# lucidrains/progen

Measured on NVIDIA H100. Metric: tokens_per_sec, higher is better.
Workload: dtype bf16

## Files before the change

### include/progen_b200.h

```cpp
#ifndef PROGEN_B200_H
#define PROGEN_B200_H
#include <stdint.h>

#ifdef __cplusplus
extern "C" {
#endif

#define PROGEN_F32 0
#define PROGEN_BF16 1

#define PROGEN_BACKEND_SIMT 0
#define PROGEN_BACKEND_TC 1

#define PROGEN_EPI_STORE 0
#define PROGEN_EPI_ROTARY 1
#define PROGEN_EPI_RESIDUAL 2
#define PROGEN_EPI_GLU 3
#define PROGEN_EPI_GELU 4
#define PROGEN_EPI_GLU_BWD 5
#define PROGEN_EPI_GELU_BWD 6
#define PROGEN_EPI_ACCUM 7

const char* progen_version(void);
const char* progen_last_error(void);
int progen_device_check(void);
long long progen_launch_count(void);

typedef struct progen_gemm_t {
  int32_t M, N, K;
  int32_t a_mn_major, b_mn_major;
  int32_t batch;
  int32_t batch_reduce;
  int32_t causal;
  int32_t split_k;
  int32_t in_dtype, out_dtype, epi_kind, backend;
  int32_t seq_len, dim_head;
  int32_t atomic, tril, tril_rows;
  int64_t lda, ldb;
  int64_t a_batch_rows, b_batch_rows, d_batch_rows;
  int64_t ldo, ldo2, ldaux;
  const void* A;
  const void* B;
  void* out;
  void* out2;
  const float* bias;
  const void* aux;
  const float* rot_sin;
  const float* rot_cos;
  float* colsum;
  int64_t lda2, ldb2;
  const void* A2;
  const void* B2;
  int32_t K2, a2_mn_major, b2_mn_major, _pad_tail;
} progen_gemm_t;

int progen_gemm(const progen_gemm_t* desc, void* stream);

int progen_embed_fwd(const int* tokens, const float* table, float* x, long long T, int d, int V, void* stream);
int progen_embed_bwd(const int* tokens, const float* dx, float* dtable, long long T, int d, int V, void* stream);

int progen_ln_shift_fwd(const void* x, long long ldx, int x_dtype, const float* scale, void* y, long long ldy, int y_dtype,
                        float* mean, float* rstd, long long T, int d, int seq_len, int shift, void* stream);
int progen_ln_shift_bwd(const void* dy, long long lddy, int act_dtype, const void* x, long long ldx, int x_dtype,
                        const float* scale, const float* mean, const float* rstd, float* dres, void* dout, long long ldo,
                        float* dscale, float* dres_colsum, long long T, int d, int seq_len, int shift, int residual,
                        void* stream);

int progen_colsum(const void* in, long long ld, int dtype, float* out, long long T, int N, void* stream);

int progen_ce_fwd_bwd(const void* logits, int dtype, const int* labels, float* weights, float* loss, void* dlogits,
                      int dlogits_dtype, int B, int n, int V, float inv_batch, void* stream);

int progen_token_logprob(const void* logits, int dtype, const int* labels, float* logp, float* seq_ll, float* seq_count,
                         int B, int n, int V, void* stream);
int progen_preference_head(const void* logits, int dtype, const int* labels, const float* ref_ll, float* logp, float* seq_ll,
                           float* seq_count, float* weights, float* stats, float* loss, float* ce_scratch, void* dlogits,
                           int dlogits_dtype, int pairs, int n, int V, float beta, float inv_pairs, void* stream);
int progen_masked_mean_pool(const void* x, long long ldx, int dtype, const int* labels, float* out, int B, int n, int d,
                            void* stream);
int progen_masked_mean_pool_bwd(const float* demb, const int* labels, void* dy, long long ldy, int dtype, int B, int n, int d,
                                void* stream);

#define PROGEN_PROPERTY_MAX_OUTPUTS 64
#define PROGEN_TASK_REGRESSION 0
#define PROGEN_TASK_CLASSIFICATION 1
int progen_property_head(const float* emb, const float* w, const float* bias, int B, int d, int C, int task, const float* y,
                         const int* cls, float inv_batch, float* pred, float* row_loss, float* loss, float* dpred, float* dw,
                         float* db, float* demb, void* stream);

// ... 121 lines not shown
```

### progen_b200/csrc/api.cu

```cuda
#include <stdarg.h>
#include "gemm.h"
#include "../../include/progen_b200.h"

static thread_local char g_err[1024] = "";
unsigned long long g_progen_launches = 0;

void progen_set_error(const char* fmt, ...) {
  va_list ap;
  va_start(ap, fmt);
  vsnprintf(g_err, sizeof(g_err), fmt, ap);
  va_end(ap);
}

extern "C" {

const char* progen_version(void) { return "progen_b200 0.1.0 (sm_90a; wgmma/TMA GEMM, CUDA " CUDA_VERSION_STR ")"; }

const char* progen_last_error(void) { return g_err; }

long long progen_launch_count(void) { return (long long)__atomic_load_n(&g_progen_launches, __ATOMIC_RELAXED); }

int progen_device_check(void) {
  int dev = 0;
  PG_CUDA(cudaGetDevice(&dev));
  cudaDeviceProp prop;
  PG_CUDA(cudaGetDeviceProperties(&prop, dev));
  if (prop.major != 9) {
    progen_set_error("device %d (%s) is sm_%d%d; libprogen_b200 is built for sm_90a only", dev, prop.name, prop.major,
                     prop.minor);
    return PROGEN_ERR_DEVICE;
  }
  return PROGEN_OK;
}

int progen_gemm(const progen_gemm_t* d, void* stream) {
  PG_CHECK_ARG(d != nullptr);
  GemmArgs g;
  g.M = d->M; g.N = d->N; g.K = d->K;
  g.A = d->A; g.lda = d->lda; g.a_mn_major = d->a_mn_major;
  g.B = d->B; g.ldb = d->ldb; g.b_mn_major = d->b_mn_major;
  g.batch = d->batch < 1 ? 1 : d->batch;
  g.a_batch_rows = d->a_batch_rows; g.b_batch_rows = d->b_batch_rows; g.d_batch_rows = d->d_batch_rows;
  g.batch_reduce = d->batch_reduce; g.causal = d->causal; g.split_k = d->split_k < 1 ? 1 : d->split_k;
  g.in_dtype = d->in_dtype; g.out_dtype = d->out_dtype; g.epi_kind = d->epi_kind;
  g.epi.out = d->out; g.epi.ldo = d->ldo; g.epi.out2 = d->out2; g.epi.ldo2 = d->ldo2;
  g.epi.bias = d->bias; g.epi.aux = d->aux; g.epi.ldaux = d->ldaux;
  g.epi.rot_sin = d->rot_sin; g.epi.rot_cos = d->rot_cos;
  g.epi.seq_len = d->seq_len > 0 ? d->seq_len : 1; g.epi.dim_head = d->dim_head > 0 ? d->dim_head : 2;
  g.epi.atomic = d->atomic; g.epi.tril = d->tril; g.epi.tril_rows = d->tril_rows > 0 ? d->tril_rows : 1;
  g.epi.colsum = d->colsum;
  g.K2 = d->K2;
  g.A2 = d->A2; g.lda2 = d->lda2; g.a2_mn_major = d->a2_mn_major;
  g.B2 = d->B2; g.ldb2 = d->ldb2; g.b2_mn_major = d->b2_mn_major;
  PG_CHECK_ARG(g.epi_kind >= 0 && g.epi_kind < EPI_NUM_KINDS);
  PG_CHECK_ARG(g.epi.out != nullptr);
  PG_CHECK_ARG(!g.epi.colsum || g.epi_kind == EPI_GLU_BWD || g.epi_kind == EPI_GELU_BWD);
  if (g.epi_kind == EPI_GLU || g.epi_kind == EPI_GELU) PG_CHECK_ARG(g.epi.bias != nullptr);
  if (g.epi_kind == EPI_GLU_BWD || g.epi_kind == EPI_GELU_BWD) PG_CHECK_ARG(g.epi.aux != nullptr);
  if (g.epi_kind == EPI_ROTARY) PG_CHECK_ARG(g.epi.rot_sin && g.epi.rot_cos && d->seq_len > 0 && d->dim_head > 0 && d->dim_head % 2 == 0);
  if (d->backend == PROGEN_BACKEND_TC) return gemm_tc_launch(g, (cudaStream_t)stream);
  if (d->backend == PROGEN_BACKEND_SIMT) return gemm_simt_launch(g, (cudaStream_t)stream);
  progen_set_error("progen_gemm: unknown backend %d", d->backend);
  return PROGEN_ERR_ARG;
}

}
```

### progen_b200/csrc/gemm.h

```cpp
#pragma once
#include "epilogues.cuh"

struct GemmArgs {
  int M, N, K;
  const void* A; long long lda; int a_mn_major;
  const void* B; long long ldb; int b_mn_major;
  int batch; long long a_batch_rows; long long b_batch_rows; long long d_batch_rows;
  int batch_reduce;
  int causal;
  int split_k;
  int in_dtype;
  int out_dtype;
  int epi_kind;
  EpiArgs epi;
  const void* A2; long long lda2; int a2_mn_major;
  const void* B2; long long ldb2; int b2_mn_major;
  int K2;
};

#define PG_CHECK_TAIL(a)                                                                                               \
  do {                                                                                                                 \
    PG_CHECK_ARG((a).K2 >= 0);                                                                                         \
    if ((a).K2 > 0) {                                                                                                  \
      PG_CHECK_ARG((a).A2 != nullptr && (a).B2 != nullptr);                                                            \
      PG_CHECK_ARG((a).split_k == 1 && !(a).causal && (a).batch == 1 && !(a).batch_reduce && (a).epi_kind != EPI_ACCUM); \
    }                                                                                                                  \
  } while (0)

int gemm_tc_launch(const GemmArgs& g, cudaStream_t stream);
int gemm_simt_launch(const GemmArgs& g, cudaStream_t stream);
```

### progen_b200/csrc/gemm_tc.cu

```cuda
#include <cuda.h>
#include <algorithm>
#include <mutex>
#include <unordered_map>
#include "gemm.h"
#include "tc_ptx.cuh"

namespace {

using namespace tc;

constexpr int BM = 128;
constexpr int BN = 128;
constexpr int BK = 64;
constexpr int WG_K = 16;
constexpr int THREADS = 384;
constexpr int A_BYTES = BM * BK * 2;
constexpr int B_BYTES = BN * BK * 2;
constexpr int STAGE_BYTES = A_BYTES + B_BYTES;
constexpr int STAGES = 4;
constexpr int EPI_ROWS = 64;
constexpr int EPI_ITEMS = EPI_ROWS * (BN / 8) / 128;
constexpr int CS_LD = BN + 4;
constexpr int CS_BYTES = EPI_ROWS * CS_LD * 4;
constexpr int SMEM_TOTAL = 1024  + STAGES * STAGE_BYTES + 2 * CS_BYTES + 2 * STAGES * 8;
static_assert(SMEM_TOTAL <= 227 * 1024, "H100: 227 KiB of shared memory per block");
constexpr int BAR_TURN = 1, BAR_EPI = 3;
constexpr int PRODUCER_REGS = 40, CONSUMER_REGS = 232;
static_assert(128 * PRODUCER_REGS + 256 * CONSUMER_REGS <= 65536, "register file");

__device__ __forceinline__ void named_bar_sync(int id, int n) { asm volatile("bar.sync %0, %1;" ::"r"(id), "r"(n) : "memory"); }
__device__ __forceinline__ void named_bar_arrive(int id, int n) { asm volatile("bar.arrive %0, %1;" ::"r"(id), "r"(n) : "memory"); }
template <int R> __device__ __forceinline__ void setmaxnreg_dec() { asm volatile("setmaxnreg.dec.sync.aligned.u32 %0;" ::"n"(R)); }
template <int R> __device__ __forceinline__ void setmaxnreg_inc() { asm volatile("setmaxnreg.inc.sync.aligned.u32 %0;" ::"n"(R)); }

struct GemmDev {
  int M, N, K;
  int batch, batch_reduce;
  int a_batch_rows, b_batch_rows;
  long long d_batch_rows;
  int causal, split_k;
  EpiArgs epi;
  int K2;
};

struct TileInfo {
  int z, m0, n0, kb_begin, kb_end;
  int kb_main;
};

template <bool TAIL>
__device__ __forceinline__ void decode_tile(const GemmDev& g, int t, TileInfo& ti) {
  const int m_tiles = (g.M + BM - 1) / BM;
  const int n_tiles = (g.N + BN - 1) / BN;
  const int per_z = g.split_k * m_tiles * n_tiles;
  ti.z = t / per_z;
  int r = t - ti.z * per_z;
  const int ks = r / (m_tiles * n_tiles);
  r -= ks * (m_tiles * n_tiles);
  ti.m0 = (r / n_tiles) * BM;
  ti.n0 = (r % n_tiles) * BN;
  const int kb_total = (g.K + BK - 1) / BK;
  int b = 0, e = kb_total;
  if (g.causal == 1) e = min(kb_total, (ti.m0 + BM + BK - 1) / BK);
  if (g.causal == 2) b = min(kb_total, ti.m0 / BK);
  if (g.split_k > 1) {
    const int per = (kb_total + g.split_k - 1) / g.split_k;
    b = min(kb_total, ks * per);
    e = min(kb_total, b + per);
  }
  ti.kb_begin = b;
  ti.kb_end = e;
  if constexpr (TAIL) {
    ti.kb_main = e;
    ti.kb_end = e + (g.K2 + BK - 1) / BK;
  }
}

template <bool A_MN, bool B_MN, int KIND, typename TO, bool TAIL>
__global__ void __launch_bounds__(THREADS, 1)
gemm_tc_kernel(const __grid_constant__ CUtensorMap tma_a, const __grid_constant__ CUtensorMap tma_b,
               const __grid_constant__ CUtensorMap tma_a2, const __grid_constant__ CUtensorMap tma_b2, const GemmDev g,
               const int tiles) {
  extern __shared__ uint8_t smem_raw[];
  const uint32_t raw_u32 = smem_u32(smem_raw);
  const uint32_t smem_base = (raw_u32 + 1023u) & ~1023u;
  const uint32_t cs_base = smem_base + STAGES * STAGE_BYTES;
  const uint32_t bar_base = cs_base + 2 * CS_BYTES;
  auto full_bar = [&](int s) { return bar_base + 8u * s; };
  auto empty_bar = [&](int s) { return bar_base + 8u * (STAGES + s); };

  const int wg = threadIdx.x >> 7;
  if (threadIdx.x == 0) {
    prefetch_tensormap(&tma_a);
    prefetch_tensormap(&tma_b);
    if constexpr (TAIL) {
      prefetch_tensormap(&tma_a2);
// ... 152 lines not shown
        const float4 x0 = *reinterpret_cast<const float4*>(cs + r * CS_LD + cc);
        const float4 x1 = *reinterpret_cast<const float4*>(cs + r * CS_LD + cc + 4);
        v[0] = x0.x; v[1] = x0.y; v[2] = x0.z; v[3] = x0.w; v[4] = x1.x; v[5] = x1.y; v[6] = x1.z; v[7] = x1.w;
        epi_finish<KIND, TO, 8>(g.epi, row_first + EPI_ROWS * h + 8 * i, col, v, cb, pre[i], col_ok && m < g.M, csum);
        if (h == 0)
          epi_load<KIND, TO, 8>(g.epi, row_first + EPI_ROWS + 8 * i, col, col_ok && m + EPI_ROWS < g.M, pre[i]);
      }
    }
    if constexpr (CS::W > 0) {
      if (g.epi.colsum) {
        constexpr int TW = 16 * CS::W;
#pragma unroll
        for (int k = 0; k < CS::W; ++k) csum[k] += __shfl_xor_sync(0xffffffffu, csum[k], 16);
        named_bar_sync(BAR_EPI + c, 128);
        if (lane < 16) {
#pragma unroll
          for (int k = 0; k < CS::W; k += 4)
            *reinterpret_cast<float4*>(cs + w * TW + lane * CS::W + k) = make_float4(csum[k], csum[k + 1], csum[k + 2], csum[k + 3]);
        }
        named_bar_sync(BAR_EPI + c, 128);
        const int out0 = CS::OUT_SCALE * ti.n0, out_cols = CS::OUT_SCALE * g.N;
#pragma unroll
        for (int q = tid; q < TW / 4; q += 128) {
          float4 s = *reinterpret_cast<const float4*>(cs + 4 * q);
#pragma unroll
          for (int ww = 1; ww < 4; ++ww) {
            const float4 x = *reinterpret_cast<const float4*>(cs + ww * TW + 4 * q);
            s.x += x.x; s.y += x.y; s.z += x.z; s.w += x.w;
          }
          if (out0 + 4 * q < out_cols)
            asm volatile("red.global.add.v4.f32 [%0], {%1, %2, %3, %4};" ::"l"(g.epi.colsum + out0 + 4 * q), "f"(s.x),
                         "f"(s.y), "f"(s.z), "f"(s.w) : "memory");
        }
      }
    }
  }
}

typedef CUresult (*EncodeTiledFn)(CUtensorMap*, CUtensorMapDataType, cuuint32_t, void*, const cuuint64_t*,
                                  const cuuint64_t*, const cuuint32_t*, const cuuint32_t*, CUtensorMapInterleave,
                                  CUtensorMapSwizzle, CUtensorMapL2promotion, CUtensorMapFloatOOBfill);

EncodeTiledFn get_encode_fn() {
  static EncodeTiledFn fn = nullptr;
  static std::once_flag once;
  std::call_once(once, [] {
    void* p = nullptr;
    cudaDriverEntryPointQueryResult q;
    if (cudaGetDriverEntryPoint("cuTensorMapEncodeTiled", &p, cudaEnableDefault, &q) == cudaSuccess &&
        q == cudaDriverEntryPointSuccess)
      fn = reinterpret_cast<EncodeTiledFn>(p);
  });
  return fn;
}

struct MapKey {
  const void* ptr; uint64_t inner, outer, stride; uint32_t box_inner, box_outer, elem_bytes, swizzle;
  bool operator==(const MapKey& o) const {
    return ptr == o.ptr && inner == o.inner && outer == o.outer && stride == o.stride && box_inner == o.box_inner &&
           box_outer == o.box_outer && elem_bytes == o.elem_bytes && swizzle == o.swizzle;
  }
};
struct MapKeyHash {
  size_t operator()(const MapKey& k) const {
    size_t h = std::hash<const void*>()(k.ptr);
    auto mix = [&](uint64_t v) { h ^= std::hash<uint64_t>()(v) + 0x9e3779b97f4a7c15ULL + (h << 6) + (h >> 2); };
// ... 19 lines not shown
  cuuint32_t box[2] = {box_inner, box_outer};
  cuuint32_t estr[2] = {1, 1};
  CUtensorMap m;
  CUresult r = fn(&m, elem_bytes == 4 ? CU_TENSOR_MAP_DATA_TYPE_FLOAT32 : CU_TENSOR_MAP_DATA_TYPE_BFLOAT16, 2,
                  const_cast<void*>(ptr), dims, strides, box, estr, CU_TENSOR_MAP_INTERLEAVE_NONE, sw, CU_TENSOR_MAP_L2_PROMOTION_L2_256B,
                  CU_TENSOR_MAP_FLOAT_OOB_FILL_NONE);
  if (r != CUDA_SUCCESS) {
    progen_set_error("cuTensorMapEncodeTiled failed (CUresult %d) ptr=%p inner=%llu outer=%llu stride=%llu box=%ux%u", (int)r,
                     ptr, (unsigned long long)inner, (unsigned long long)outer, (unsigned long long)row_stride_elems,
                     box_inner, box_outer);
    return PROGEN_ERR_CUDA;
  }
  if (cache.size() > 4096) cache.clear();
  cache.emplace(key, m);
  *out = m;
  return PROGEN_OK;
}


template <bool A_MN, bool B_MN, int KIND, typename TO, bool TAIL>
int launch_inst(const CUtensorMap& ta, const CUtensorMap& tb, const CUtensorMap& ta2, const CUtensorMap& tb2,
                const GemmDev& gd, int tiles, cudaStream_t stream) {
  auto kern = gemm_tc_kernel<A_MN, B_MN, KIND, TO, TAIL>;
  static bool attr_set = false;
  if (!attr_set) {
    PG_CUDA(cudaFuncSetAttribute(kern, cudaFuncAttributeMaxDynamicSharedMemorySize, SMEM_TOTAL));
    attr_set = true;
  }
  kern<<<std::min(tiles, pg_num_sms()), THREADS, SMEM_TOTAL, stream>>>(ta, tb, ta2, tb2, gd, tiles);
  PG_LAUNCH_CHECK();
  return PROGEN_OK;
}

}

int pg_tensor_map_2d_bf16(const void* ptr, uint64_t inner, uint64_t outer, uint64_t row_stride_elems, uint32_t box_inner,
                          uint32_t box_outer, CUtensorMap* out) {
  return get_tensor_map(ptr, inner, outer, row_stride_elems, box_inner, box_outer, out);
}

int gemm_tc_launch(const GemmArgs& a, cudaStream_t stream) {
  PG_CHECK_ARG(a.in_dtype == PG_BF16);
  PG_CHECK_ARG(a.M > 0 && a.N > 0 && a.K > 0 && a.batch >= 1 && a.split_k >= 1);
  PG_CHECK_ARG(a.N % 8 == 0);
  PG_CHECK_ARG(a.K % BK == 0);
  PG_CHECK_ARG(a.lda % 8 == 0 && a.ldb % 8 == 0);
  PG_CHECK_ARG((reinterpret_cast<uintptr_t>(a.A) & 15) == 0 && (reinterpret_cast<uintptr_t>(a.B) & 15) == 0);
  PG_CHECK_ARG(!(a.split_k > 1 && a.causal));
  if (a.epi_kind == EPI_ROTARY) PG_CHECK_ARG(a.epi.seq_len % 32 == 0);
  PG_CHECK_ARG((reinterpret_cast<uintptr_t>(a.epi.colsum) & 15) == 0);
  PG_CHECK_ARG(!(a.split_k > 1 || a.batch_reduce) || (a.epi_kind == EPI_ACCUM && a.epi.atomic));
  PG_CHECK_TAIL(a);
  const bool tail = a.K2 > 0;
  if (tail) {
    PG_CHECK_ARG(a.K2 % 8 == 0 && a.lda2 % 8 == 0 && a.ldb2 % 8 == 0);
    PG_CHECK_ARG(a.a2_mn_major == a.a_mn_major && a.b2_mn_major == a.b_mn_major);
    PG_CHECK_ARG((reinterpret_cast<uintptr_t>(a.A2) & 15) == 0 && (reinterpret_cast<uintptr_t>(a.B2) & 15) == 0);
  }

  const uint64_t a_rows = (a.batch > 1 && a.a_batch_rows > 0) ? (uint64_t)a.a_batch_rows * a.batch
                                                              : (uint64_t)(a.a_mn_major ? a.K : a.M);
  const uint64_t b_rows = (a.batch > 1 && a.b_batch_rows > 0) ? (uint64_t)a.b_batch_rows * a.batch
                                                              : (uint64_t)(a.b_mn_major ? a.K : a.N);
  CUtensorMap ta, tb;
  int rc;
  if (!a.a_mn_major) rc = get_tensor_map(a.A, a.K, a_rows, a.lda, BK, BM, &ta);
  else               rc = get_tensor_map(a.A, a.M, a_rows, a.lda, 64, BK, &ta);
  if (rc) return rc;
  if (!a.b_mn_major) rc = get_tensor_map(a.B, a.K, b_rows, a.ldb, BK, BN, &tb);
  else               rc = get_tensor_map(a.B, a.N, b_rows, a.ldb, 64, BK, &tb);
  if (rc) return rc;
  CUtensorMap ta2 = ta, tb2 = tb;
  if (tail) {
    if (!a.a_mn_major) rc = get_tensor_map(a.A2, a.K2, a.M, a.lda2, BK, BM, &ta2);
    else               rc = get_tensor_map(a.A2, a.M, a.K2, a.lda2, 64, BK, &ta2);
    if (rc) return rc;
    if (!a.b_mn_major) rc = get_tensor_map(a.B2, a.K2, a.N, a.ldb2, BK, BN, &tb2);
    else               rc = get_tensor_map(a.B2, a.N, a.K2, a.ldb2, 64, BK, &tb2);
    if (rc) return rc;
  }

  GemmDev gd;
  gd.M = a.M; gd.N = a.N; gd.K = a.K;
  gd.batch = a.batch; gd.batch_reduce = a.batch_reduce;
  gd.a_batch_rows = (int)a.a_batch_rows; gd.b_batch_rows = (int)a.b_batch_rows; gd.d_batch_rows = a.d_batch_rows;
  gd.causal = a.causal; gd.split_k = a.split_k;
  gd.epi = a.epi;
  gd.K2 = a.K2;
  const long long tiles = (long long)a.batch * a.split_k * ((a.M + BM - 1) / BM) * ((a.N + BN - 1) / BN);
  PG_CHECK_ARG(tiles < (1ll << 31));

  const int am = a.a_mn_major ? 1 : 0, bm = a.b_mn_major ? 1 : 0;
  const bool obf = a.out_dtype == PG_BF16;
#define TC_CASE(AM, BMJ, KIND, TO)                                                                       \
  return tail ? launch_inst<AM, BMJ, KIND, TO, true>(ta, tb, ta2, tb2, gd, (int)tiles, stream)            \
              : launch_inst<AM, BMJ, KIND, TO, false>(ta, tb, ta2, tb2, gd, (int)tiles, stream)
  switch (a.epi_kind) {
    case EPI_STORE:
      if (!am && bm) { if (obf) TC_CASE(false, true, EPI_STORE, bf16); else TC_CASE(false, true, EPI_STORE, float); }
      if (!am && !bm) { if (obf) TC_CASE(false, false, EPI_STORE, bf16); else TC_CASE(false, false, EPI_STORE, float); }
      if (am && bm) { if (obf) TC_CASE(true, true, EPI_STORE, bf16); else TC_CASE(true, true, EPI_STORE, float); }
      break;
    case EPI_ROTARY:
      if (!am && bm && obf) TC_CASE(false, true, EPI_ROTARY, bf16);
      break;
    case EPI_RESIDUAL:
      if (!am && bm) TC_CASE(false, true, EPI_RESIDUAL, float);
      break;
    case EPI_GLU:
      if (!am && bm && obf) TC_CASE(false, true, EPI_GLU, bf16);
      break;
    case EPI_GELU:
      if (!am && bm && obf) TC_CASE(false, true, EPI_GELU, bf16);
      break;
    case EPI_GLU_BWD:
      if (!am && !bm && obf) TC_CASE(false, false, EPI_GLU_BWD, bf16);
      break;
    case EPI_GELU_BWD:
      if (!am && !bm && obf) TC_CASE(false, false, EPI_GELU_BWD, bf16);
      break;
    case EPI_ACCUM:
      if (am && bm) return launch_inst<true, true, EPI_ACCUM, float, false>(ta, tb, ta2, tb2, gd, (int)tiles, stream);
      if (!am && !bm) return launch_inst<false, false, EPI_ACCUM, float, false>(ta, tb, ta2, tb2, gd, (int)tiles, stream);
      break;
    default: break;
  }
// ... 5 lines not shown
```

### progen_b200/engine.py

```python
import math
import numpy as np
import torch

from . import lib as L

P = 'pro_gen_base/~/'
ALIGN = 64


CUT_ALIGN = 128


def counted_length(labels):
    labels = np.asarray(labels)
    n = labels.shape[1]
    pad = labels == 0
    first = np.where(pad.any(1), pad.argmax(1), n)
    last = np.where((~pad).any(1), n - 1 - (~pad)[:, ::-1].argmax(1), -1)
    return np.minimum(n, np.maximum(first, last) + 1)


def cut_length(labels):
    n = np.asarray(labels).shape[1]
    need = int(counted_length(labels).max()) if len(labels) else 1
    return min(n, -(-need // CUT_ALIGN) * CUT_ALIGN)


def layer_kinds(depth, global_mlp_depth, ff_glu):
    out = []
    for i in range(depth):
        use_gmlp = (depth - i) <= global_mlp_depth
        out.append('sgu' if use_gmlp else ('glu' if ff_glu else 'gelu'))
# ... 20 lines not shown
        a = P + f'attn{i}/~/'
        specs += [ParamSpec(a + 'layer_norm', 'scale', (d,)),
                  ParamSpec(a + 'linear', 'w', (d, 3 * inner)),
                  ParamSpec(a + 'linear_1', 'w', (inner, d)), ParamSpec(a + 'linear_1', 'b', (d,))]
        f = P + f'ff{i}/~/'
        h_in = hid * 2 if kind == 'glu' else hid
        h_out = hid // 2 if kind == 'sgu' else hid
        glu = kind == 'glu'
        specs += [ParamSpec(f + 'layer_norm', 'scale', (d,)),
                  ParamSpec(f + 'linear', 'w', (d, h_in), interleave=glu), ParamSpec(f + 'linear', 'b', (h_in,), interleave=glu)]
        if kind == 'sgu':
            half = hid // 2
            specs += [ParamSpec(f + 'sgu/~/layer_norm', 'scale', (half,)),
                      ParamSpec(f + 'sgu', 'spatial_weights', (n, n)), ParamSpec(f + 'sgu', 'spatial_biases', (n, 1)),
                      ParamSpec(f + 'sgu/~/linear', 'w', (half, half)), ParamSpec(f + 'sgu/~/linear', 'b', (half,))]
        specs += [ParamSpec(f + 'linear_1', 'w', (h_out, d)), ParamSpec(f + 'linear_1', 'b', (d,))]
    specs += [ParamSpec(P + 'layer_norm', 'scale', (d,)),
              ParamSpec(P + 'linear', 'w', (d, V)), ParamSpec(P + 'linear', 'b', (V,))]
    off = 0
    for s in [s for s in specs if s.decay] + [s for s in specs if not s.decay]:
        s.offset = off
        off += (s.size + ALIGN - 1) // ALIGN * ALIGN
    n_decay = sum((s.size + ALIGN - 1) // ALIGN * ALIGN for s in specs if s.decay)
    return specs, off, n_decay


def _interleave(a):
    H = a.shape[-1] // 2
    return np.stack((a[..., :H], a[..., H:]), axis=-1).reshape(a.shape)


def _deinterleave(a):
    return np.concatenate((a[..., 0::2], a[..., 1::2]), axis=-1)


class Acts:

    def __init__(self, B, T, tok, labels, X, lay, meanf, rstdf, yf, logits, inplace=False, rows=None, res=None):
        self.B, self.T, self.tok, self.labels, self.X, self.lay = B, T, tok, labels, X, lay
        self.meanf, self.rstdf, self.yf, self.logits = meanf, rstdf, yf, logits
        self.inplace = inplace
        self.rows = rows
        self.res = res

    def view(self, B, n):
        T = B * n
        cut = lambda t: None if t is None else t[:T]
        return Acts(B, T, cut(self.tok), cut(self.labels), [cut(x) for x in self.X],
                    [{k: cut(v) for k, v in s.items()} for s in self.lay], cut(self.meanf), cut(self.rstdf), cut(self.yf),
                    cut(self.logits), self.inplace, None if self.rows is None else self.rows[:B], self.res)


class Engine:
    def __init__(self, cfg, mixed_precision=False, device=None):
        L.require_device()
        self.cfg = cfg
        self.dev = torch.device('cuda', torch.cuda.current_device()) if device is None else torch.device(device)
        self.mp = bool(mixed_precision)
        self.act = torch.bfloat16 if self.mp else torch.float32
        self.act_dt = L.BF16 if self.mp else L.F32
        self.backend = L.BACKEND_TC if self.mp else L.BACKEND_SIMT
        self.kinds = layer_kinds(cfg['depth'], cfg['global_mlp_depth'], cfg['ff_glu'])
        self.attn_tc = self.attn_wgmma = self.mp
        d, n, w = cfg['dim'], cfg['seq_len'], cfg['window_size']
        self.d, self.n, self.w, self.V = d, n, w, cfg['num_tokens']
        self.h, self.dh = cfg['heads'], cfg['dim_head']
# ... 184 lines not shown

    def lora_fwd(self, x, K, module, N):
        lo = self.lora
        if lo is None:
            return {}
        u = lo.u[module]
        self.fwd_gemm(x, K, lo.seg(lo.lp, module, 'lora_a'), lo.r, u)
        return dict(A2=u, lda2=lo.r, B2=lo.seg(lo.lp, module, 'lora_b'), ldb2=N, K2=lo.r)

    def lora_bwd(self, x, K, module, dy, N):
        lo = self.lora
        if lo is None:
            return {}
        g, A = lo.g, lo.seg(lo.lp, module, 'lora_a')
        self.dgrad_gemm(dy, N, lo.seg(lo.lp, module, 'lora_b'), lo.r, g)
        self.wgrad_gemm(lo.u[module], lo.r, dy, N, lo.seg(lo.grads, module, 'lora_b'))
        self.wgrad_gemm(x, K, g, lo.r, lo.seg(lo.grads, module, 'lora_a'))
        return dict(A2=g, lda2=lo.r, B2=A, ldb2=lo.r, K2=lo.r)

    def fwd_gemm(self, x, K, w, N, out, epi=L.EPI_STORE, out_dtype=None, acts=None, **kw):
        self._mm(M=(acts or self.acts).T, N=N, K=K, A=x, lda=K, B=w, ldb=N, b_mn=True, out=out, ldo=kw.pop('ldo', N), epi=epi,
                 out_dtype=self.act_dt if out_dtype is None else out_dtype, **kw)

    def dgrad_gemm(self, dy, N_out, w, K_in, out, epi=L.EPI_STORE, **kw):
        self._mm(M=self.T, N=K_in, K=N_out, A=dy, lda=N_out, B=w, ldb=N_out, out=out, ldo=kw.pop('ldo', K_in), epi=epi,
                 out_dtype=self.act_dt, **kw)

    def wgrad_gemm(self, x, K_in, dy, N_out, dw):
        split = self.wgrad_split(K_in, N_out) if self.backend == L.BACKEND_TC else 1
        self._mm(M=K_in, N=N_out, K=self.T, A=x, lda=K_in, a_mn=True, B=dy, ldb=N_out, b_mn=True, out=dw, ldo=N_out,
                 epi=L.EPI_ACCUM, out_dtype=L.F32, split_k=split, atomic=split > 1)

    def wgrad_split(self, K_in, N_out):
        tiles = ((K_in + 127) // 128) * ((N_out + 127) // 128)
        fill = lambda s: tiles * s / (-(-tiles * s // self.num_sms) * self.num_sms)
        return max(range(1, min(8, max(1, self.T // 64)) + 1), key=lambda s: (round(fill(s), 6), -s))

    def colsum(self, t, N, out, ld=None):
        L.check(self.lib.progen_colsum(t.data_ptr(), N if ld is None else ld, L.dt(t), out.data_ptr(), self.T, N, L.stream()), 'colsum')

    def ln_fwd(self, x, ldx, scale, y, ldy, mean, rstd, dcols, shift, acts=None, seq_len=None):
        L.check(self.lib.progen_ln_shift_fwd(x.data_ptr(), ldx, L.dt(x), scale.data_ptr(), y.data_ptr(), ldy, L.dt(y),
                                             mean.data_ptr(), rstd.data_ptr(), (acts or self.acts).T, dcols,
                                             self.n if seq_len is None else seq_len, int(shift), L.stream()), 'ln_fwd')

    def forward(self, ids):
        B = ids.shape[0]
        self.ensure_batch(B)
        self.tok.copy_(torch.as_tensor(ids).reshape(-1).to(device=self.dev, dtype=torch.int32), non_blocking=True)
        self._forward_device()
        return self.logits

    def prefill(self, ids, P, sink):
        Bs = ids.shape[0]
        if tuple(ids.shape[1:]) != (self.n,) or not 0 < P < self.n:
            raise L.ProgenError(f'prefill: ids must be (B, {self.n}) and 0 < P < {self.n}')
        acts = self.inference_acts(Bs)
        acts.tok.copy_(torch.as_tensor(ids).reshape(-1).to(device=self.dev, dtype=torch.int32))
        self._forward_device(acts, sink=lambda i, name, buf: sink(i, name, buf, P))

    def _forward_device(self, acts=None, sink=None, length=None, logits=True):
        acts = self.acts if acts is None else acts
        lib, st = self.lib, L.stream()
        cfg, d, I, hid, T = self.cfg, self.d, self.I, self.hid, acts.T
        n = self.n if length is None else length
        if T != acts.B * n:
            raise L.ProgenError(f'forward: {T} token rows are not {acts.B} rows of length {n}')
        shift = cfg['shift_tokens']
        lo = self.lora if acts is self.acts else None
# ... 355 lines not shown
```

### progen_b200/lib.py

```python
import ctypes as C
import os
import torch

F32, BF16 = 0, 1
BACKEND_SIMT, BACKEND_TC = 0, 1
EPI_STORE, EPI_ROTARY, EPI_RESIDUAL, EPI_GLU, EPI_GELU, EPI_GLU_BWD, EPI_GELU_BWD, EPI_ACCUM = range(8)
TASK_REGRESSION, TASK_CLASSIFICATION = 0, 1
PROPERTY_MAX_OUTPUTS = 64

_HERE = os.path.dirname(os.path.abspath(__file__))
LIB_PATH = os.path.join(_HERE, 'libprogen_b200.so')


class ProgenError(RuntimeError):
    pass


class GemmDesc(C.Structure):
    _fields_ = [
        ('M', C.c_int32), ('N', C.c_int32), ('K', C.c_int32),
        ('a_mn_major', C.c_int32), ('b_mn_major', C.c_int32),
        ('batch', C.c_int32), ('batch_reduce', C.c_int32), ('causal', C.c_int32), ('split_k', C.c_int32),
        ('in_dtype', C.c_int32), ('out_dtype', C.c_int32), ('epi_kind', C.c_int32), ('backend', C.c_int32),
        ('seq_len', C.c_int32), ('dim_head', C.c_int32),
        ('atomic', C.c_int32), ('tril', C.c_int32), ('tril_rows', C.c_int32),
        ('lda', C.c_int64), ('ldb', C.c_int64),
        ('a_batch_rows', C.c_int64), ('b_batch_rows', C.c_int64), ('d_batch_rows', C.c_int64),
        ('ldo', C.c_int64), ('ldo2', C.c_int64), ('ldaux', C.c_int64),
        ('A', C.c_void_p), ('B', C.c_void_p), ('out', C.c_void_p), ('out2', C.c_void_p),
        ('bias', C.c_void_p), ('aux', C.c_void_p), ('rot_sin', C.c_void_p), ('rot_cos', C.c_void_p),
        ('colsum', C.c_void_p),
        ('lda2', C.c_int64), ('ldb2', C.c_int64), ('A2', C.c_void_p), ('B2', C.c_void_p),
        ('K2', C.c_int32), ('a2_mn_major', C.c_int32), ('b2_mn_major', C.c_int32), ('_pad_tail', C.c_int32),
    ]


_lib = None

_LL, _I, _P, _F = C.c_longlong, C.c_int, C.c_void_p, C.c_float

PROTOTYPES = {
    'progen_version': [],
    'progen_last_error': [],
    'progen_device_check': [],
    'progen_launch_count': [],
    'progen_gemm': [C.POINTER(GemmDesc), _P],
    'progen_embed_fwd': [_P, _P, _P, _LL, _I, _I, _P],
    'progen_embed_bwd': [_P, _P, _P, _LL, _I, _I, _P],
    'progen_ln_shift_fwd': [_P, _LL, _I, _P, _P, _LL, _I, _P, _P, _LL, _I, _I, _I, _P],
    'progen_ln_shift_bwd': [_P, _LL, _I, _P, _LL, _I, _P, _P, _P, _P, _P, _LL, _P, _P, _LL, _I, _I, _I, _I, _P],
    'progen_colsum': [_P, _LL, _I, _P, _LL, _I, _P],
    'progen_ce_fwd_bwd': [_P, _I, _P, _P, _P, _P, _I, _I, _I, _I, _F, _P],
    'progen_token_logprob': [_P, _I, _P, _P, _P, _P, _I, _I, _I, _P],
    'progen_preference_head': [_P, _I, _P, _P, _P, _P, _P, _P, _P, _P, _P, _P, _I, _I, _I, _I, _F, _F, _P],
    'progen_masked_mean_pool': [_P, _LL, _I, _P, _P, _I, _I, _I, _P],
    'progen_masked_mean_pool_bwd': [_P, _P, _P, _LL, _I, _I, _I, _I, _P],
    'progen_property_head': [_P, _P, _P, _I, _I, _I, _I, _P, _P, _F, _P, _P, _P, _P, _P, _P, _P, _P],
    'progen_rotary_bwd': [_P, _LL, _I, _P, _P, _LL, _I, _I, _I, _P],
    'progen_local_attn_fwd_simt': [_P, _P, _P, _I, _I, _I, _I, _I, _I, _P],
    'progen_local_attn_bwd_simt': [_P, _P, _P, _P, _P, _P, _I, _I, _I, _I, _I, _I, _P],
    'progen_local_attn_fwd_tc': [_P, _P, _P, _I, _I, _I, _I, _I, _P],
    'progen_local_attn_bwd_tc': [_P, _P, _P, _P, _P, _P, _P, _P, _I, _I, _I, _I, _I, _P],
    'progen_sgu_gate_fwd': [_P, _LL, _P, _LL, _P, _P, _LL, _I, _LL, _I, _I, _P],
    'progen_sgu_gate_bwd': [_P, _LL, _P, _LL, _P, _LL, _P, _P, _LL, _P, _LL, _P, _I, _LL, _I, _I, _P],
    'progen_gelu_bwd': [_P, _P, _I, _LL, _P],
    'progen_cast_f32': [_P, _P, _I, _LL, _P],
    'progen_scale_cast_f32': [_P, _P, _I, _F, _LL, _P],
    'progen_tril_cast': [_P, _P, _I, _I, _P],
    'progen_decode_run': [_P, _P],
    'progen_gather_rows_f32': [_P, _LL, _I, _I, _LL, _P, _I, _I, _I, _I, _I, _I, _P, _LL, _LL, _LL, _P],
    'progen_optim_workspace_floats': [],
    'progen_grad_sqnorm': [_P, _LL, _P, _P, _P],
    'progen_adamw_step': [_P, _P, _P, _P, _P, _P, _LL, _LL, _P, _F, _F, _F, _F, _F, _F, _LL, _I, _P],
    'progen_adamw_step_dev': [_P, _P, _P, _P, _P, _P, _LL, _LL, _P, _F, _F, _F, _F, _F, _F, _I, _P, _P],
}
_RESTYPES = {'progen_version': C.c_char_p, 'progen_last_error': C.c_char_p, 'progen_launch_count': C.c_longlong}


def load():
# ... 13 lines not shown


def version():
    return load().progen_version().decode()


def check(rc, what=''):
    if rc != 0:
        raise ProgenError(f'{what} failed (code {rc}): {load().progen_last_error().decode()}')


def require_device():
    if not torch.cuda.is_available():
        raise ProgenError('no CUDA device: progen_b200 has no CPU fallback (sm_90a only)')
    check(load().progen_device_check(), 'progen_device_check')


def dt(t):
    if t.dtype == torch.float32:
        return F32
    if t.dtype == torch.bfloat16:
        return BF16
    raise ProgenError(f'unsupported dtype {t.dtype}')


def ptr(t):
    return 0 if t is None else t.data_ptr()


def stream():
    return torch.cuda.current_stream().cuda_stream


def gemm(*, M, N, K, A, lda, B, ldb, out, ldo, epi=EPI_STORE, backend, a_mn=False, b_mn=False, in_dtype, out_dtype=F32,
         batch=1, a_batch_rows=0, b_batch_rows=0, d_batch_rows=0, batch_reduce=False, causal=0, split_k=1,
         out2=None, ldo2=0, bias=None, aux=None, ldaux=0, rot_sin=None, rot_cos=None, seq_len=0, dim_head=0,
         atomic=False, tril=False, tril_rows=0, colsum=None, A2=None, lda2=0, a2_mn=None, B2=None, ldb2=0, b2_mn=None, K2=0):
    d = GemmDesc()
    d.M, d.N, d.K = M, N, K
    d.a_mn_major, d.b_mn_major = int(a_mn), int(b_mn)
    d.batch, d.batch_reduce, d.causal, d.split_k = batch, int(batch_reduce), causal, split_k
    d.in_dtype, d.out_dtype, d.epi_kind, d.backend = in_dtype, out_dtype, epi, backend
    d.seq_len, d.dim_head = seq_len, dim_head
    d.atomic, d.tril, d.tril_rows = int(atomic), int(tril), tril_rows
    d.lda, d.ldb = lda, ldb
    d.a_batch_rows, d.b_batch_rows, d.d_batch_rows = a_batch_rows, b_batch_rows, d_batch_rows
    d.ldo, d.ldo2, d.ldaux = ldo, ldo2, ldaux
    as_ptr = lambda x: x if isinstance(x, int) else ptr(x)
    d.A, d.B, d.out, d.out2 = as_ptr(A), as_ptr(B), as_ptr(out), as_ptr(out2)
    d.bias, d.aux, d.rot_sin, d.rot_cos = as_ptr(bias), as_ptr(aux), as_ptr(rot_sin), as_ptr(rot_cos)
    d.colsum = as_ptr(colsum)
    if K2:
        d.K2, d.lda2, d.ldb2, d.A2, d.B2 = K2, lda2, ldb2, as_ptr(A2), as_ptr(B2)
        d.a2_mn_major = int(a_mn if a2_mn is None else a2_mn)
        d.b2_mn_major = int(b_mn if b2_mn is None else b2_mn)
    check(load().progen_gemm(C.byref(d), stream()), 'progen_gemm')
```

Measured before the change: 1.026 million.

## Add 256x128 wide-tile TC GEMM path with automatic tile selection

Adds a second warp-specialized tensor-core GEMM kernel that uses a 256-row M tile. Each of two consumer warpgroups computes a 128x128 slab, so every loaded B tile is reused across twice as many rows. The host picks this tile automatically for large-K plain-store or accumulate GEMMs such as weight gradients, and the weight-gradient split-k choice now accounts for the chosen tile size. In exchange the kernel needs more shared memory, uses a lag barrier to stagger the two consumers, and fewer tiles can leave SMs underfilled.

```diff
diff --git a/include/progen_b200.h b/include/progen_b200.h
--- a/include/progen_b200.h
+++ b/include/progen_b200.h
@@ -51,10 +51,12 @@
   int64_t lda2, ldb2;
   const void* A2;
   const void* B2;
-  int32_t K2, a2_mn_major, b2_mn_major, _pad_tail;
+  int32_t K2, a2_mn_major, b2_mn_major;
+  int32_t tile;
 } progen_gemm_t;
 
 int progen_gemm(const progen_gemm_t* desc, void* stream);
+int progen_gemm_tile_m(const progen_gemm_t* desc);
 
 int progen_embed_fwd(const int* tokens, const float* table, float* x, long long T, int d, int V, void* stream);
 int progen_embed_bwd(const int* tokens, const float* dx, float* dtable, long long T, int d, int V, void* stream);
diff --git a/progen_b200/csrc/api.cu b/progen_b200/csrc/api.cu
--- a/progen_b200/csrc/api.cu
+++ b/progen_b200/csrc/api.cu
@@ -33,8 +33,7 @@
   return PROGEN_OK;
 }
 
-int progen_gemm(const progen_gemm_t* d, void* stream) {
-  PG_CHECK_ARG(d != nullptr);
+static GemmArgs gemm_args(const progen_gemm_t* d) {
   GemmArgs g;
   g.M = d->M; g.N = d->N; g.K = d->K;
   g.A = d->A; g.lda = d->lda; g.a_mn_major = d->a_mn_major;
@@ -52,6 +51,13 @@
   g.K2 = d->K2;
   g.A2 = d->A2; g.lda2 = d->lda2; g.a2_mn_major = d->a2_mn_major;
   g.B2 = d->B2; g.ldb2 = d->ldb2; g.b2_mn_major = d->b2_mn_major;
+  g.tile = d->tile;
+  return g;
+}
+
+int progen_gemm(const progen_gemm_t* d, void* stream) {
+  PG_CHECK_ARG(d != nullptr);
+  const GemmArgs g = gemm_args(d);
   PG_CHECK_ARG(g.epi_kind >= 0 && g.epi_kind < EPI_NUM_KINDS);
   PG_CHECK_ARG(g.epi.out != nullptr);
   PG_CHECK_ARG(!g.epi.colsum || g.epi_kind == EPI_GLU_BWD || g.epi_kind == EPI_GELU_BWD);
@@ -64,4 +70,9 @@
   return PROGEN_ERR_ARG;
 }
 
+int progen_gemm_tile_m(const progen_gemm_t* d) {
+  PG_CHECK_ARG(d != nullptr && d->backend == PROGEN_BACKEND_TC);
+  return gemm_tc_tile_m(gemm_args(d));
 }
+
+}
diff --git a/progen_b200/csrc/gemm.h b/progen_b200/csrc/gemm.h
--- a/progen_b200/csrc/gemm.h
+++ b/progen_b200/csrc/gemm.h
@@ -16,6 +16,7 @@
   const void* A2; long long lda2; int a2_mn_major;
   const void* B2; long long ldb2; int b2_mn_major;
   int K2;
+  int tile;
 };
 
 #define PG_CHECK_TAIL(a)                                                                                               \
@@ -28,4 +29,5 @@
   } while (0)
 
 int gemm_tc_launch(const GemmArgs& g, cudaStream_t stream);
+int gemm_tc_tile_m(const GemmArgs& g);
 int gemm_simt_launch(const GemmArgs& g, cudaStream_t stream);
diff --git a/progen_b200/csrc/gemm_tc.cu b/progen_b200/csrc/gemm_tc.cu
--- a/progen_b200/csrc/gemm_tc.cu
+++ b/progen_b200/csrc/gemm_tc.cu
@@ -48,20 +48,20 @@
   int kb_main;
 };
 
-template <bool TAIL>
+template <bool TAIL, int TILE_M = BM>
 __device__ __forceinline__ void decode_tile(const GemmDev& g, int t, TileInfo& ti) {
-  const int m_tiles = (g.M + BM - 1) / BM;
+  const int m_tiles = (g.M + TILE_M - 1) / TILE_M;
   const int n_tiles = (g.N + BN - 1) / BN;
   const int per_z = g.split_k * m_tiles * n_tiles;
   ti.z = t / per_z;
   int r = t - ti.z * per_z;
   const int ks = r / (m_tiles * n_tiles);
   r -= ks * (m_tiles * n_tiles);
-  ti.m0 = (r / n_tiles) * BM;
+  ti.m0 = (r / n_tiles) * TILE_M;
   ti.n0 = (r % n_tiles) * BN;
   const int kb_total = (g.K + BK - 1) / BK;
   int b = 0, e = kb_total;
-  if (g.causal == 1) e = min(kb_total, (ti.m0 + BM + BK - 1) / BK);
+  if (g.causal == 1) e = min(kb_total, (ti.m0 + TILE_M + BK - 1) / BK);
   if (g.causal == 2) b = min(kb_total, ti.m0 / BK);
   if (g.split_k > 1) {
     const int per = (kb_total + g.split_k - 1) / g.split_k;
@@ -280,6 +280,163 @@
             asm volatile("red.global.add.v4.f32 [%0], {%1, %2, %3, %4};" ::"l"(g.epi.colsum + out0 + 4 * q), "f"(s.x),
                          "f"(s.y), "f"(s.z), "f"(s.w) : "memory");
         }
+      }
+    }
+  }
+}
+
+constexpr int W_BM = 256;
+constexpr int W_A_BYTES = W_BM * BK * 2;
+constexpr int W_STAGE_BYTES = W_A_BYTES + B_BYTES;
+constexpr int W_STAGES = 4;
+constexpr int W_CS_ROWS = 8;
+constexpr int W_CS_BYTES = W_CS_ROWS * CS_LD * 4;
+constexpr int W_SMEM_TOTAL = 1024  + W_STAGES * W_STAGE_BYTES + 8 * W_CS_BYTES + 2 * W_STAGES * 8;
+static_assert(W_SMEM_TOTAL <= 227 * 1024, "H100: 227 KiB of shared memory per block");
+constexpr int W_MIN_KBLOCKS = 64;
+constexpr int W_LAG = 2, BAR_LAG = 1;
+static_assert(W_LAG < W_STAGES, "consumer 0 must reach the lag barrier without a stage release from consumer 1");
+
+template <bool A_MN, bool B_MN, int KIND, typename TO>
+__global__ void __launch_bounds__(THREADS, 1)
+gemm_tc_wide_kernel(const __grid_constant__ CUtensorMap tma_a, const __grid_constant__ CUtensorMap tma_b, const GemmDev g,
+                    const int tiles) {
+  static_assert(KIND == EPI_STORE || KIND == EPI_ACCUM, "plain epilogues only");
+  extern __shared__ uint8_t smem_raw[];
+  const uint32_t raw_u32 = smem_u32(smem_raw);
+  const uint32_t smem_base = (raw_u32 + 1023u) & ~1023u;
+  const uint32_t cs_base = smem_base + W_STAGES * W_STAGE_BYTES;
+  const uint32_t bar_base = cs_base + 8 * W_CS_BYTES;
+  auto full_bar = [&](int s) { return bar_base + 8u * s; };
+  auto empty_bar = [&](int s) { return bar_base + 8u * (W_STAGES + s); };
+
+  const int wg = threadIdx.x >> 7;
+  if (threadIdx.x == 0) {
+    prefetch_tensormap(&tma_a);
+    prefetch_tensormap(&tma_b);
+    for (int s = 0; s < W_STAGES; ++s) {
+      mbar_init(full_bar(s), 1);
+      mbar_init(empty_bar(s), 2);
+    }
+    fence_barrier_init();
+  }
+  __syncthreads();
+
+  int stage = 0;
+  uint32_t phase = 0;
+  auto advance = [&] {
+    if (++stage == W_STAGES) { stage = 0; phase ^= 1u; }
+  };
+
+  if (wg == 0) {
+    setmaxnreg_dec<PRODUCER_REGS>();
+    if (threadIdx.x == 0) {
+      for (int t = blockIdx.x; t < tiles; t += gridDim.x) {
+        TileInfo ti;
+        decode_tile<false, W_BM>(g, t, ti);
+        for (int kb = ti.kb_begin; kb < ti.kb_end; ++kb) {
+          mbar_wait(empty_bar(stage), phase ^ 1);
+          const uint32_t sa = smem_base + stage * W_STAGE_BYTES;
+          const uint32_t sb = sa + W_A_BYTES;
+          mbar_expect_tx(full_bar(stage), W_STAGE_BYTES);
+          const int k0 = kb * BK;
+          if constexpr (!A_MN) {
+#pragma unroll
+            for (int i = 0; i < W_BM / BM; ++i)
+              tma_load_2d(sa + i * A_BYTES, &tma_a, full_bar(stage), k0, ti.m0 + BM * i);
+          } else {
+#pragma unroll
+            for (int i = 0; i < W_BM / 64; ++i)
+              tma_load_2d(sa + i * 8192, &tma_a, full_bar(stage), ti.m0 + 64 * i, k0);
+          }
+          if constexpr (!B_MN) {
+            tma_load_2d(sb, &tma_b, full_bar(stage), k0, ti.n0);
+          } else {
+#pragma unroll
+            for (int i = 0; i < BN / 64; ++i) tma_load_2d(sb + i * 8192, &tma_b, full_bar(stage), ti.n0 + 64 * i, k0);
+          }
+          advance();
+        }
+      }
+    }
+    return;
+  }
+
+  setmaxnreg_inc<CONSUMER_REGS>();
+  const int c = wg - 1;
+  const int tid = threadIdx.x & 127;
+  const int w = tid >> 5, lane = tid & 31;
+  float* cs = reinterpret_cast<float*>(smem_raw + (cs_base - raw_u32)) + (4 * c + w) * (W_CS_BYTES / 4);
+  bool lag_open = c == 0;
+  if (c == 1) named_bar_sync(BAR_LAG, 256);
+  for (int t = blockIdx.x; t < tiles; t += gridDim.x) {
+    TileInfo ti;
+    decode_tile<false, W_BM>(g, t, ti);
+    float acc[2][64];
+#pragma unroll
+    for (int i = 0; i < 64; ++i) acc[0][i] = acc[1][i] = 0.f;
+    int prev = -1;
+    for (int kb = ti.kb_begin; kb < ti.kb_end; ++kb) {
+      mbar_wait(full_bar(stage), phase);
+      const uint32_t sa = smem_base + stage * W_STAGE_BYTES + c * A_BYTES;
+      const uint64_t adesc0 = make_smem_desc<A_MN>(sa), adesc1 = make_smem_desc<A_MN>(sa + 8192);
+      const uint64_t bdesc = make_smem_desc<B_MN>(smem_base + stage * W_STAGE_BYTES + W_A_BYTES);
+      constexpr uint32_t a_step = A_MN ? (2048 >> 4) : (32 >> 4), b_step = B_MN ? (2048 >> 4) : (32 >> 4);
+      fence_regs(acc[0]);
+      fence_regs(acc[1]);
+      wgmma_fence();
+#pragma unroll
+      for (int k = 0; k < BK / WG_K; ++k) {
+        wgmma_m64n128k16_bf16<A_MN ? 1 : 0, B_MN ? 1 : 0>(acc[0], adesc0 + (uint64_t)(k * a_step), bdesc + (uint64_t)(k * b_step));
+        wgmma_m64n128k16_bf16<A_MN ? 1 : 0, B_MN ? 1 : 0>(acc[1], adesc1 + (uint64_t)(k * a_step), bdesc + (uint64_t)(k * b_step));
+      }
+      wgmma_commit();
+      fence_regs(acc[0]);
+      fence_regs(acc[1]);
+      wgmma_wait<1>();
+      if (prev >= 0 && tid == 0) mbar_arrive(empty_bar(prev));
+      prev = stage;
+      advance();
+      if (lag_open && kb + 1 - ti.kb_begin == W_LAG) {
+        named_bar_arrive(BAR_LAG, 256);
+        lag_open = false;
+      }
+    }
+    if (lag_open) {
+      named_bar_arrive(BAR_LAG, 256);
+      lag_open = false;
+    }
+    wgmma_wait<0>();
+    fence_regs(acc[0]);
+    fence_regs(acc[1]);
+    if (prev >= 0 && tid == 0) mbar_arrive(empty_bar(prev));
+
+    const int cc = 8 * (lane & 15), col = ti.n0 + cc;
+    const bool col_ok = col < g.N;
+    EpiCol<8> cb;
+    EpiPre<KIND, TO, 8> pre;
+    float csum[1];
+    epi_load_col<KIND, 8>(g.epi, col, col_ok, cb);
+#pragma unroll
+    for (int h = 0; h < 2; ++h) {
+#pragma unroll
+      for (int e = 0; e < 2; ++e) {
+#pragma unroll
+        for (int j = 0; j < BN / 8; ++j)
+          *reinterpret_cast<float2*>(cs + (lane >> 2) * CS_LD + 8 * j + 2 * (lane & 3)) =
+              make_float2(acc[h][4 * j + 2 * e], acc[h][4 * j + 2 * e + 1]);
+        __syncwarp();
+#pragma unroll
+        for (int i = 0; i < W_CS_ROWS * (BN / 8) / 32; ++i) {
+          const int r = 2 * i + (lane >> 4);
+          const int m = ti.m0 + 128 * c + 64 * h + 16 * w + 8 * e + r;
+          float v[8];
+          const float4 x0 = *reinterpret_cast<const float4*>(cs + r * CS_LD + cc);
+          const float4 x1 = *reinterpret_cast<const float4*>(cs + r * CS_LD + cc + 4);
+          v[0] = x0.x; v[1] = x0.y; v[2] = x0.z; v[3] = x0.w; v[4] = x1.x; v[5] = x1.y; v[6] = x1.z; v[7] = x1.w;
+          epi_finish<KIND, TO, 8>(g.epi, (long long)m, col, v, cb, pre, col_ok && m < g.M, csum);
+        }
+        __syncwarp();
       }
     }
   }
@@ -365,6 +522,37 @@
   return PROGEN_OK;
 }
 
+template <bool A_MN, bool B_MN, int KIND, typename TO>
+int launch_wide(const CUtensorMap& ta, const CUtensorMap& tb, const GemmDev& gd, int tiles, cudaStream_t stream) {
+  auto kern = gemm_tc_wide_kernel<A_MN, B_MN, KIND, TO>;
+  static bool attr_set = false;
+  if (!attr_set) {
+    PG_CUDA(cudaFuncSetAttribute(kern, cudaFuncAttributeMaxDynamicSharedMemorySize, W_SMEM_TOTAL));
+    attr_set = true;
+  }
+  kern<<<std::min(tiles, pg_num_sms()), THREADS, W_SMEM_TOTAL, stream>>>(ta, tb, gd, tiles);
+  PG_LAUNCH_CHECK();
+  return PROGEN_OK;
+}
+
+}
+
+int gemm_tc_tile_m(const GemmArgs& a) {
+  const bool eligible = (a.epi_kind == EPI_STORE || a.epi_kind == EPI_ACCUM) && a.K2 == 0 && a.batch == 1 &&
+                        !a.batch_reduce && !a.causal && a.a_mn_major == a.b_mn_major;
+  if (a.tile == 1) return BM;
+  if (a.tile == 2) {
+    if (eligible) return W_BM;
+    progen_set_error("gemm_tc: the 256 x 128 tile takes EPI_STORE / EPI_ACCUM, operands of one major, no tail, batch 1, "
+                     "not causal (epi=%d a_mn=%d b_mn=%d K2=%d batch=%d causal=%d)", a.epi_kind, a.a_mn_major,
+                     a.b_mn_major, a.K2, a.batch, a.causal);
+    return PROGEN_ERR_UNSUPPORTED;
+  }
+  PG_CHECK_ARG(a.tile == 0);
+  if (!eligible || a.M < W_BM || a.split_k < 1) return BM;
+  const int kb_unit = ((a.K + BK - 1) / BK + a.split_k - 1) / a.split_k;
+  const long long units = (long long)a.split_k * ((a.M + W_BM - 1) / W_BM) * ((a.N + BN - 1) / BN);
+  return kb_unit >= W_MIN_KBLOCKS && 2 * units > pg_num_sms() ? W_BM : BM;
 }
 
 int pg_tensor_map_2d_bf16(const void* ptr, uint64_t inner, uint64_t outer, uint64_t row_stride_elems, uint32_t box_inner,
@@ -413,6 +601,9 @@
     if (rc) return rc;
   }
 
+  const int tile_m = gemm_tc_tile_m(a);
+  if (tile_m < 0) return tile_m;
+
   GemmDev gd;
   gd.M = a.M; gd.N = a.N; gd.K = a.K;
   gd.batch = a.batch; gd.batch_reduce = a.batch_reduce;
@@ -420,11 +611,20 @@
   gd.causal = a.causal; gd.split_k = a.split_k;
   gd.epi = a.epi;
   gd.K2 = a.K2;
-  const long long tiles = (long long)a.batch * a.split_k * ((a.M + BM - 1) / BM) * ((a.N + BN - 1) / BN);
+  const long long tiles = (long long)a.batch * a.split_k * ((a.M + tile_m - 1) / tile_m) * ((a.N + BN - 1) / BN);
   PG_CHECK_ARG(tiles < (1ll << 31));
 
   const int am = a.a_mn_major ? 1 : 0, bm = a.b_mn_major ? 1 : 0;
   const bool obf = a.out_dtype == PG_BF16;
+  if (tile_m == W_BM) {
+#define TC_WIDE(AM, KIND, TO) return launch_wide<AM, AM, KIND, TO>(ta, tb, gd, (int)tiles, stream)
+    if (a.epi_kind == EPI_ACCUM) {
+      if (am) TC_WIDE(true, EPI_ACCUM, float); else TC_WIDE(false, EPI_ACCUM, float);
+    }
+    if (am) { if (obf) TC_WIDE(true, EPI_STORE, bf16); else TC_WIDE(true, EPI_STORE, float); }
+    if (obf) TC_WIDE(false, EPI_STORE, bf16); else TC_WIDE(false, EPI_STORE, float);
+#undef TC_WIDE
+  }
 #define TC_CASE(AM, BMJ, KIND, TO)                                                                       \
   return tail ? launch_inst<AM, BMJ, KIND, TO, true>(ta, tb, ta2, tb2, gd, (int)tiles, stream)            \
               : launch_inst<AM, BMJ, KIND, TO, false>(ta, tb, ta2, tb2, gd, (int)tiles, stream)
diff --git a/progen_b200/engine.py b/progen_b200/engine.py
--- a/progen_b200/engine.py
+++ b/progen_b200/engine.py
@@ -1,3 +1,4 @@
+import functools
 import math
 import numpy as np
 import torch
@@ -84,6 +85,16 @@
 
 def _deinterleave(a):
     return np.concatenate((a[..., 0::2], a[..., 1::2]), axis=-1)
+
+
+@functools.lru_cache(maxsize=None)
+def _wgrad_split(K_in, N_out, T, num_sms):
+    def key(s):
+        tm = L.gemm_tile_m(M=K_in, N=N_out, K=T, lda=K_in, a_mn=True, ldb=N_out, b_mn=True, epi=L.EPI_ACCUM,
+                           backend=L.BACKEND_TC, in_dtype=L.BF16, split_k=s, atomic=s > 1)
+        units = -(-K_in // tm) * -(-N_out // 128) * s
+        return round(units / (-(-units // num_sms) * num_sms), 6), tm, -s
+    return max(range(1, min(8, max(1, T // 64)) + 1), key=key)
 
 
 class Acts:
@@ -334,9 +345,7 @@
                  epi=L.EPI_ACCUM, out_dtype=L.F32, split_k=split, atomic=split > 1)
 
     def wgrad_split(self, K_in, N_out):
-        tiles = ((K_in + 127) // 128) * ((N_out + 127) // 128)
-        fill = lambda s: tiles * s / (-(-tiles * s // self.num_sms) * self.num_sms)
-        return max(range(1, min(8, max(1, self.T // 64)) + 1), key=lambda s: (round(fill(s), 6), -s))
+        return _wgrad_split(K_in, N_out, self.T, self.num_sms)
 
     def colsum(self, t, N, out, ld=None):
         L.check(self.lib.progen_colsum(t.data_ptr(), N if ld is None else ld, L.dt(t), out.data_ptr(), self.T, N, L.stream()), 'colsum')
diff --git a/progen_b200/lib.py b/progen_b200/lib.py
--- a/progen_b200/lib.py
+++ b/progen_b200/lib.py
@@ -31,7 +31,7 @@
         ('bias', C.c_void_p), ('aux', C.c_void_p), ('rot_sin', C.c_void_p), ('rot_cos', C.c_void_p),
         ('colsum', C.c_void_p),
         ('lda2', C.c_int64), ('ldb2', C.c_int64), ('A2', C.c_void_p), ('B2', C.c_void_p),
-        ('K2', C.c_int32), ('a2_mn_major', C.c_int32), ('b2_mn_major', C.c_int32), ('_pad_tail', C.c_int32),
+        ('K2', C.c_int32), ('a2_mn_major', C.c_int32), ('b2_mn_major', C.c_int32), ('tile', C.c_int32),
     ]
 
 
@@ -45,6 +45,7 @@
     'progen_device_check': [],
     'progen_launch_count': [],
     'progen_gemm': [C.POINTER(GemmDesc), _P],
+    'progen_gemm_tile_m': [C.POINTER(GemmDesc)],
     'progen_embed_fwd': [_P, _P, _P, _LL, _I, _I, _P],
     'progen_embed_bwd': [_P, _P, _P, _LL, _I, _I, _P],
     'progen_ln_shift_fwd': [_P, _LL, _I, _P, _P, _LL, _I, _P, _P, _LL, _I, _I, _I, _P],
@@ -124,10 +125,21 @@
     return torch.cuda.current_stream().cuda_stream
 
 
-def gemm(*, M, N, K, A, lda, B, ldb, out, ldo, epi=EPI_STORE, backend, a_mn=False, b_mn=False, in_dtype, out_dtype=F32,
-         batch=1, a_batch_rows=0, b_batch_rows=0, d_batch_rows=0, batch_reduce=False, causal=0, split_k=1,
-         out2=None, ldo2=0, bias=None, aux=None, ldaux=0, rot_sin=None, rot_cos=None, seq_len=0, dim_head=0,
-         atomic=False, tril=False, tril_rows=0, colsum=None, A2=None, lda2=0, a2_mn=None, B2=None, ldb2=0, b2_mn=None, K2=0):
+def gemm(**kw):
+    check(load().progen_gemm(C.byref(gemm_desc(**kw)), stream()), 'progen_gemm')
+
+
+def gemm_tile_m(**kw):
+    rc = load().progen_gemm_tile_m(C.byref(gemm_desc(**kw)))
+    check(min(rc, 0), 'progen_gemm_tile_m')
+    return rc
+
+
+def gemm_desc(*, M, N, K, A=0, lda, B=0, ldb, out=0, ldo=0, epi=EPI_STORE, backend, a_mn=False, b_mn=False, in_dtype,
+              out_dtype=F32, batch=1, a_batch_rows=0, b_batch_rows=0, d_batch_rows=0, batch_reduce=False, causal=0, split_k=1,
+              out2=None, ldo2=0, bias=None, aux=None, ldaux=0, rot_sin=None, rot_cos=None, seq_len=0, dim_head=0,
+              atomic=False, tril=False, tril_rows=0, colsum=None, A2=None, lda2=0, a2_mn=None, B2=None, ldb2=0, b2_mn=None,
+              K2=0, tile=0):
     d = GemmDesc()
     d.M, d.N, d.K = M, N, K
     d.a_mn_major, d.b_mn_major = int(a_mn), int(b_mn)
@@ -146,4 +158,5 @@
         d.K2, d.lda2, d.ldb2, d.A2, d.B2 = K2, lda2, ldb2, as_ptr(A2), as_ptr(B2)
         d.a2_mn_major = int(a_mn if a2_mn is None else a2_mn)
         d.b2_mn_major = int(b_mn if b2_mn is None else b2_mn)
-    check(load().progen_gemm(C.byref(d), stream()), 'progen_gemm')
+    d.tile = tile
+    return d
```

New measurement: 1.051 million, median of 6. 1.02x the previous value.
